# AILab-CVC/SEED-X

Measured on AMD Instinct MI355X. Metric: end-to-end generations/sec (img-in -> txt + 1024px-img-out), higher is better.
Workload: dtype fp16

## Files before the change

### include/seedx_hip.h

```cpp
#ifndef SEEDX_HIP_H
#define SEEDX_HIP_H
#include <stdint.h>
#ifdef __cplusplus
extern "C" {
#endif

#define SX_OK 0
#define SX_ERR_INVALID 1
#define SX_ERR_HIP 2

#define SX_F16 0
#define SX_BF16 1
#define SX_F32 2
#define SX_BF16X3 3
#define SX_F16X2 4
#define SX_FP8_E4M3 5
#define SX_FP4_E2M1 6
#define SX_TILED16 0x100

#define SX_ACT_NONE 0
#define SX_ACT_GELU 1
#define SX_ACT_SILU 2

#define SX_A_LINEAR 0
// ... 8 lines not shown
  void* C;
  const float* bias;
  const float* bias2d;
  const float* residual;
  int32_t M, N, K;
  int32_t ldc, ldr;
  int32_t n_valid;
  int32_t res_mod;
  int32_t bias2d_rows;
  int32_t dtype;
  int32_t out_dtype;
  int32_t act;
  int32_t glu;
  int32_t a_mode;
  int32_t B, Hin, Win, Cin, Hout, Wout;
  int32_t stride;
  int32_t upsample;
  int32_t ld_bias2d;
  int32_t pad_mode;
  int32_t a_planes;
} sx_gemm_args;
int sx_gemm(const sx_gemm_args* args, void* stream);
int sx_gemm_gn(const sx_gemm_args* args, double* stats, int groups, int rows_per_sample, int* fused_host, void* stream);
typedef struct sx_gemm_ln_args {
  void* x16_out;
  double* row_stats_out;
  const double* row_stats_in;
  const float* colsum;
  int32_t ld_x16;
  int32_t dim;
  float eps;
  int32_t reserved;
} sx_gemm_ln_args;
int sx_gemm_ln(const sx_gemm_args* args, const sx_gemm_ln_args* ln, void* stream);
int sx_gemm_force_tile(int cfg);
int sx_gemm_debug_stamps(void* buf);
int sx_gemm_pick_tile(int M, int N, int K, int glu, int conv);

typedef struct sx_gemv_args {
  const void* x;
  const void* W;
  void* y;
  const float* residual;
  int32_t M, N, K;
  int32_t dtype, out_dtype, act, glu;
  int32_t w_layout;
// ... 346 lines not shown
```

### seed-x_amd/_lib.py

```python
import ctypes as C
import os

_HERE = os.path.dirname(os.path.abspath(__file__))
LIB_PATH = os.path.join(_HERE, "lib", "libseedx_hip.so")

SX_F16, SX_BF16, SX_F32 = 0, 1, 2
SX_BF16X3 = 3
SX_F16X2 = 4
SX_FP8_E4M3 = 5
SX_FP4_E2M1 = 6
SX_TILED16 = 0x100
SX_ACT_NONE, SX_ACT_GELU, SX_ACT_SILU = 0, 1, 2
SX_A_LINEAR, SX_A_CONV3X3 = 0, 1

c_i32, c_i64, c_f32, c_vp = C.c_int32, C.c_int64, C.c_float, C.c_void_p


class GemmArgs(C.Structure):
    _fields_ = [("A", c_vp), ("W", c_vp), ("C", c_vp), ("bias", c_vp), ("bias2d", c_vp), ("residual", c_vp),
                ("M", c_i32), ("N", c_i32), ("K", c_i32), ("ldc", c_i32), ("ldr", c_i32), ("n_valid", c_i32),
                ("res_mod", c_i32), ("bias2d_rows", c_i32), ("dtype", c_i32), ("out_dtype", c_i32),
                ("act", c_i32), ("glu", c_i32), ("a_mode", c_i32),
                ("B", c_i32), ("Hin", c_i32), ("Win", c_i32), ("Cin", c_i32), ("Hout", c_i32), ("Wout", c_i32),
                ("stride", c_i32), ("upsample", c_i32), ("ld_bias2d", c_i32), ("pad_mode", c_i32), ("a_planes", c_i32)]
# ... 92 lines not shown
    _fields_ = [("Q", c_vp), ("K", c_vp), ("V", c_vp), ("O", c_vp),
                ("B", c_i32), ("H", c_i32), ("Sq", c_i32), ("Skv", c_i32), ("D", c_i32), ("reserved", c_i32),
                ("q_batch_stride", c_i64), ("q_row_stride", c_i64), ("q_head_stride", c_i64),
                ("k_batch_stride", c_i64), ("k_row_stride", c_i64), ("k_head_stride", c_i64),
                ("v_batch_stride", c_i64), ("v_row_stride", c_i64), ("v_head_stride", c_i64),
                ("o_batch_stride", c_i64), ("o_row_stride", c_i64),
                ("scale", c_f32), ("causal", c_i32), ("dtype", c_i32)]


class AttnSmallArgs(C.Structure):
    _fields_ = [("Q", c_vp), ("K", c_vp), ("V", c_vp), ("O", c_vp),
                ("B", c_i32), ("H", c_i32), ("Sq", c_i32), ("Skv", c_i32), ("D", c_i32),
                ("q_batch_stride", c_i64), ("q_row_stride", c_i64), ("q_head_stride", c_i64),
                ("k_batch_stride", c_i64), ("k_row_stride", c_i64), ("k_head_stride", c_i64),
                ("v_batch_stride", c_i64), ("v_row_stride", c_i64), ("v_head_stride", c_i64),
                ("o_batch_stride", c_i64), ("o_row_stride", c_i64),
                ("scale", c_f32), ("dtype", c_i32)]


SIGNATURES = {
    "sx_version": [],
    "sx_gemm": [C.POINTER(GemmArgs), c_vp],
    "sx_gemm_gn": [C.POINTER(GemmArgs), c_vp, c_i32, c_i32, C.POINTER(c_i32), c_vp],
    "sx_gemm_ln": [C.POINTER(GemmArgs), C.POINTER(GemmLnArgs), c_vp],
    "sx_gemm_force_tile": [c_i32],
    "sx_gemm_debug_stamps": [c_vp],
    "sx_gemm_pick_tile": [c_i32, c_i32, c_i32, c_i32, c_i32],
    "sx_gemv": [C.POINTER(GemvArgs), c_vp],
    "sx_gemv_ssq_parts": [c_i32, c_i32, c_i32],
    "sx_gemv_plan": [C.POINTER(GemvArgs), C.POINTER(c_i32)],
    "sx_gemv_force_valu": [c_i32],
    "sx_layernorm": [c_vp, c_i32, c_vp, c_i32, c_vp, c_vp, c_i32, c_i32, c_f32, c_i32, c_vp],
    "sx_softmax_rows": [c_vp, c_i64, c_vp, c_i64, c_i32, c_i32, c_f32, c_i32, c_vp],
    "sx_groupnorm": [c_vp, c_vp, c_vp, c_i32, c_vp, c_vp, c_vp, c_i32, c_i32, c_i32, c_i32, c_f32, c_i32, c_vp],
    "sx_groupnorm2": [c_vp, c_vp, c_i32, c_vp, c_vp, c_i32, c_vp, c_vp, c_vp, c_i32, c_i32, c_i32, c_i32, c_f32, c_i32, c_vp],
    "sx_groupnorm_sp": [c_vp, c_vp, c_i32, c_vp, c_vp, c_i32, c_vp, c_vp, c_vp, c_i32, c_i32, c_i32, c_i32, c_i32, c_f32, c_i32,
                        c_i32, c_vp],
    "sx_attention": [C.POINTER(AttnArgs), c_vp],
    "sx_norm_tune": [c_i32, c_i32],
    "sx_gemv_tune": [c_i32, c_i32],
    "sx_comm_alloc": [C.POINTER(c_vp), C.c_uint64],
    "sx_comm_free": [c_vp],
    "sx_ipc_export": [c_vp, C.c_char_p],
    "sx_ipc_open": [C.c_char_p, C.POINTER(c_vp)],
    "sx_ipc_close": [c_vp],
    "sx_allreduce_oneshot": [C.POINTER(OneshotArgs), c_vp],
# ... 94 lines not shown
```

### seed-x_amd/csrc/gemm.hip

```cpp
#include "gemm_common.h"

namespace sxk_gemm {

template <typename TT, int BM, int BN, int WM, int WN, int NSTAGE, int AMODE>
__global__ __launch_bounds__(WM * WN * 64) void gemm_kernel(const GemmP p) {
#if defined(__HIP_DEVICE_COMPILE__)
  typedef typename TT::vec8 vec8;
  constexpr int NW = WM * WN;
  static_assert(NW == 4 || NW == 8, "4 or 8 waves per block");
  constexpr int TM = BM / WM, TN = BN / WN;
  constexpr int FM = TM / 16, FN = TN / 16;
  constexpr bool kGlu = (FN % 2 == 0);
  constexpr int BNP = (BN + 8 * NW - 1) / (8 * NW) * (8 * NW);
  constexpr int A_PER_WAVE = BM / (8 * NW);
  constexpr int B_PER_WAVE = BNP / (8 * NW);
  constexpr int LOADS = A_PER_WAVE + B_PER_WAVE;
  constexpr int A_BYTES = BM * 128, B_BYTES = BNP * 128, STAGE = A_BYTES + B_BYTES;
  static_assert(LOADS * (NSTAGE - 1) <= 63, "vmcnt range");
  extern __shared__ __attribute__((aligned(16))) unsigned char smem[];

  const int tid = threadIdx.x, lane = tid & 63;
  const int wave = __builtin_amdgcn_readfirstlane(tid >> 6);
  const int wm = wave / WN, wn = wave % WN;
  unsigned long long t_start = 0, t_first = 0, t_main = 0;
// ... 377 lines not shown
  GemmP p;
  memset(&p, 0, sizeof(p));
  p.A = a->A; p.W = a->W; p.C = a->C; p.bias = a->bias; p.bias2d = a->bias2d; p.residual = a->residual;
  SX_CHECK(a->a_planes >= 0 && a->a_planes <= 2, "sx_gemm: a_planes=%d", a->a_planes);
  const int planes = a->a_planes == 2 ? 2 : 1;
  SX_CHECK(planes == 1 || (a->a_mode == SX_A_LINEAR && !ln), "sx_gemm: a_planes = 2 is for plain linear GEMMs");
  const int Kk = a->K * planes;
  p.M = a->M; p.N = a->N; p.K = Kk; p.Kw = a->K; p.ldc = a->ldc; p.ldr = a->ldr; p.res_mod = a->res_mod;
  p.n_valid = a->n_valid > 0 ? a->n_valid : n_out;
  p.bias2d_rows = a->bias2d_rows; p.out_dtype = a->out_dtype; p.act = a->act; p.glu = a->glu;
  p.ldb2 = a->ld_bias2d > 0 ? a->ld_bias2d : a->N;
  p.pad = 1;
  uint64_t a_bytes;
  const bool phases = a->a_mode == SX_A_CONV3X3 && a->upsample == 2;
  if (a->a_mode == SX_A_CONV3X3) {
    SX_CHECK(a->upsample >= 0 && a->upsample <= 2, "sx_gemm conv: upsample=%d", a->upsample);
    SX_CHECK(a->Cin % 64 == 0 && a->K == (phases ? 4 : 9) * a->Cin, "sx_gemm conv: Cin=%d K=%d", a->Cin, a->K);
    SX_CHECK(a->stride == 1 || a->stride == 2, "sx_gemm conv: stride");
    if (phases) {
      SX_CHECK(a->stride == 1 && a->pad_mode == 0, "sx_gemm conv: upsample = 2 is stride 1, pad 1");
      SX_CHECK((int64_t)a->B * a->Hin * a->Win % 256 == 0,
               "sx_gemm conv: upsample = 2 needs B*Hin*Win %% 256 == 0 (B=%d Hin=%d Win=%d): a 256-row tile must not straddle a phase",
               a->B, a->Hin, a->Win);
      SX_CHECK(!a->residual && !gn_stats, "sx_gemm conv: upsample = 2 takes no residual and no GroupNorm statistics");
    }
    SX_CHECK(a->M == a->B * a->Hout * a->Wout, "sx_gemm conv: M != B*Hout*Wout");
    const int hv = a->upsample ? 2 * a->Hin : a->Hin, wv = a->upsample ? 2 * a->Win : a->Win;
    SX_CHECK(a->pad_mode == 0 || a->pad_mode == 1, "sx_gemm conv: pad_mode");
    const int padsum = a->pad_mode ? 1 : 2;
    SX_CHECK(a->Hout == (hv + padsum - 3) / a->stride + 1 && a->Wout == (wv + padsum - 3) / a->stride + 1,
             "sx_gemm conv: output geometry mismatch");
    p.pad = a->pad_mode ? 0 : 1;
    p.Hin = a->Hin; p.Win = a->Win; p.Cin = a->Cin; p.Hout = a->Hout; p.Wout = a->Wout;
    p.stride = a->stride; p.upsample = a->upsample;
    a_bytes = (uint64_t)a->B * a->Hin * a->Win * a->Cin * 2;
  } else {
    SX_CHECK(a->a_mode == SX_A_LINEAR, "sx_gemm: bad a_mode");
    a_bytes = (uint64_t)a->M * Kk * 2;
  }
  const uint64_t w_bytes = (uint64_t)a->N * a->K * 2 * (phases ? 4 : 1);
  SX_CHECK(a_bytes < 0x7fffffffull && w_bytes < 0x7fffffffull, "sx_gemm: operand exceeds 2 GiB descriptor range");
  p.a_bytes = (unsigned)a_bytes;
  p.w_bytes = (unsigned)w_bytes;
  hipStream_t st = (hipStream_t)stream;
  p.res_init = (p.residual && p.act == SX_ACT_NONE && !p.glu) ? 1 : 0;
  if (ln) {
    SX_CHECK(a->a_mode == SX_A_LINEAR && !gn_stats, "sx_gemm_ln: linear GEMMs only");
// ... 6 lines not shown
    } else {
      SX_CHECK(ln->colsum && ln->dim == a->K && ln->eps > 0.f, "sx_gemm_ln consumer: colsum / dim (= K) / eps");
      SX_CHECK(a->out_dtype == a->dtype && !a->residual && !a->bias2d, "sx_gemm_ln consumer: 16-bit output, no residual / bias2d");
      p.ln_in = ln->row_stats_in; p.ln_cs = ln->colsum; p.ln_eps = ln->eps; p.ln_inv_dim = 1.0f / (float)ln->dim;
    }
  }
  unsigned allow = 0x7f;
  if (ln || phases) allow = 0;
  allow |= pp_supported(p, a->dtype, 256, a->a_mode) ? 0x80u : 0u;
  allow |= pp_supported(p, a->dtype, 320, a->a_mode) ? 0x100u : 0u;
  SX_CHECK(!(g_force_tile == 7 || g_force_tile == 8) || ((allow >> g_force_tile) & 1u),
           "sx_gemm: forced ping-pong tile has no kernel for this epilogue");
  if (ln) {
    const int plain = pick_tile(a->M, a->N, Kk, a->glu != 0, false, g_force_tile, 0x1ff);
    SX_CHECK((plain == 7 || plain == 8) && ((allow >> plain) & 1u),
             "sx_gemm_ln: M=%d N=%d K=%d does not run on a ping-pong tile with this epilogue (tile %d): keep sx_layernorm for it", a->M,
             a->N, a->K, plain);
    allow = 1u << plain;
  }
  SX_CHECK(!phases || allow, "sx_gemm conv: upsample = 2 has no ping-pong kernel for this epilogue");
  const int force = (phases && g_force_tile != 7 && g_force_tile != 8) ? -1 : g_force_tile;
  const int cfg = pick_tile(a->M, a->N, Kk, a->glu != 0, a->a_mode == SX_A_CONV3X3, force, allow);
  if (cfg == 7 || cfg == 8) {
    if (gn_stats && a->out_dtype == SX_F32 && !a->glu && a->act == SX_ACT_NONE && p.n_valid == a->N && a->N % gn_groups == 0 &&
        (a->N / gn_groups) % 2 == 0 && gn_rows % 256 == 0 && a->M % gn_rows == 0) {
      p.gn_stats = gn_stats; p.gn_groups = gn_groups; p.gn_cpg = a->N / gn_groups; p.gn_rows = gn_rows;
      *gn_fused = 1;
    }
    return launch_pp(p, a->dtype, cfg == 7 ? 256 : 320, a->a_mode, st);
  }
#define SX_GEMM_DISPATCH(TT)                                                  \
  switch (cfg) {                                                              \
    case 0: return launch_cfg<TT, 128, 128, 2, 2, 2>(p, a->a_mode, st);       \
    case 1: return launch_cfg<TT, 128, 80, 4, 1, 3>(p, a->a_mode, st);        \
    case 2: return launch_cfg<TT, 64, 128, 2, 2, 3>(p, a->a_mode, st);        \
    case 3: return launch_cfg<TT, 64, 64, 2, 2, 3>(p, a->a_mode, st);         \
    case 4: return launch_cfg<TT, 256, 256, 2, 4, 2>(p, a->a_mode, st);       \
    case 5: return launch_cfg<TT, 256, 320, 2, 4, 2>(p, a->a_mode, st);       \
    default: return launch_cfg<TT, 256, 160, 4, 2, 2>(p, a->a_mode, st);      \
  }
  if (a->dtype == SX_BF16) { SX_GEMM_DISPATCH(BF16) } else { SX_GEMM_DISPATCH(F16) }
#undef SX_GEMM_DISPATCH
}
```

### seed-x_amd/csrc/gemm_pp.hip

```cpp
#include "gemm_common.h"
#include <type_traits>

namespace sxk_gemm {

#define SX_A_CONV3X3_UP 2
#define SX_A_CONV3X3_PH 3

#define PP_SYNC()                            \
  do {                                       \
    __builtin_amdgcn_sched_barrier(0);       \
    __builtin_amdgcn_s_barrier();            \
    __builtin_amdgcn_sched_barrier(0);       \
  } while (0)

template <typename TT, int BN, int AMODE, bool OUT32, int ACT, bool GLU, int LN = 0>
__global__ __launch_bounds__(512) void gemm_pp_kernel(const GemmP p) {
#if defined(__HIP_DEVICE_COMPILE__)
  typedef typename TT::vec8 vec8;
  static_assert(LN != 2 || (OUT32 && !GLU && ACT == SX_ACT_NONE), "the LayerNorm producer is the plain fp32-output epilogue");
  constexpr int BM = 256, TN = BN / 4, FN = TN / 16, FM = 8, FH = 4;
  constexpr int NB = BN / 64;
  constexpr int C1 = NB - 3, C2 = 3;
  constexpr int WAITN = 4 + NB;
  constexpr int A_BYTES = BM * 128, STAGE = A_BYTES + BN * 128;
// ... 442 lines not shown
      x += __builtin_bit_cast(float, __builtin_amdgcn_update_dpp(0, __builtin_bit_cast(int, x), 0x140, 0xF, 0xF, true));
      return x;
    };
#pragma unroll
    for (int i = 0; i < FN; ++i) {
      gsl[i] = row16_sum(gsl[i]);
      gql[i] = row16_sum(gql[i]);
      gsh[i] = row16_sum(gsh[i]);
      gqh[i] = row16_sum(gqh[i]);
    }
    float* gslot = (float*)smem;
    const int gbase = n0 / p.gn_cpg;
    const int nlast = (n0 + BN < p.N ? n0 + BN : p.N) - 1;
    const int ngr = nlast / p.gn_cpg - gbase + 1;
    __syncthreads();
    if ((lane & 15) == 0) {
#pragma unroll
      for (int i = 0; i < FN; ++i) {
        const int cp = (wc * TN + i * 16 + lq) >> 1;
        *(f32x4_t*)(gslot + ((size_t)g * (BN / 2) + cp) * 2) = (f32x4_t){gsl[i], gql[i], gsh[i], gqh[i]};
      }
    }
    __syncthreads();
    const int smp = m0 / p.gn_rows;
    for (int t = tid; t < 2 * ngr; t += 512) {
      const int G = gbase + (t >> 1), which = t & 1;
      int c_lo = G * p.gn_cpg - n0, c_hi = (G + 1) * p.gn_cpg - n0;
      c_lo = c_lo < 0 ? 0 : c_lo;
      const int c_end = (p.N - n0 < BN ? p.N - n0 : BN);
      c_hi = c_hi > c_end ? c_end : c_hi;
      float acc = 0.f;
      for (int cp = c_lo >> 1; cp < (c_hi >> 1); ++cp) acc += gslot[(size_t)cp * 2 + which];
      for (int cp = c_lo >> 1; cp < (c_hi >> 1); ++cp) acc += gslot[((size_t)(BN / 2) + cp) * 2 + which];
      atomicAdd(&p.gn_stats[((size_t)smp * p.gn_groups + G) * 2 + which], (double)acc);
    }
  }
  if (p.dbg) {
    asm volatile("s_waitcnt vmcnt(0)" ::: "memory");
    const unsigned long long t_end = __builtin_amdgcn_s_memtime();
    if (tid == 0) {
      unsigned long long* d = p.dbg + (size_t)blockIdx.x * 4;
      d[0] = t_start; d[1] = t_first; d[2] = t_main; d[3] = t_end;
    }
  }
#endif
}

// ... 128 lines not shown
```

### seed-x_amd/ops.py

```python
import contextlib
import ctypes as C
import gc
import math

import os

import torch

from . import _lib
from ._lib import (SX_A_CONV3X3, SX_A_LINEAR, SX_ACT_GELU, SX_ACT_NONE, SX_ACT_SILU, SX_BF16, SX_F16, SX_F32,
                   AttnArgs, AttnSmallArgs, GemmArgs, GemvArgs, check)

_DT = {torch.float16: SX_F16, torch.bfloat16: SX_BF16, torch.float32: SX_F32}
_TD = {v: k for k, v in _DT.items()}
ACT = {None: SX_ACT_NONE, "none": SX_ACT_NONE, "gelu": SX_ACT_GELU, "silu": SX_ACT_SILU}


def dt_code(dtype):
    return _DT[dtype]


def _stream():
    return C.c_void_p(torch.cuda.current_stream().cuda_stream)

# ... 7 lines not shown


@contextlib.contextmanager
def graph_capture(g):
    gc.collect()
    was = gc.isenabled()
    gc.disable()
    try:
        with torch.cuda.graph(g):
            yield
    finally:
        if was:
            gc.enable()


def _f32c(t):
    if t is None:
        return None
    assert t.dtype == torch.float32 and t.is_contiguous(), "expected contiguous fp32 tensor"
    return t


class GnStats:
    __slots__ = ("buf", "groups", "rows", "ready")

    def __init__(self, buf, groups, rows):
        self.buf, self.groups, self.rows, self.ready = buf, int(groups), int(rows), False

    @staticmethod
    def arena(n, B, groups, device):
        return torch.zeros((n, B, groups, 2), dtype=torch.float64, device=device)


class LnRows:
    __slots__ = ("x16", "stats")

    def __init__(self, M, C, dtype, device, stats=None):
        self.x16 = torch.empty((M, C), dtype=dtype, device=device)
        self.stats = stats if stats is not None else torch.zeros((M, 2), dtype=torch.float64, device=device)
        assert self.stats.shape == (M, 2) and self.stats.dtype == torch.float64 and self.stats.is_contiguous()


def gemm_tile(M, N, K, glu=False, conv=False):
    return int(_lib.load().sx_gemm_pick_tile(int(M), int(N), int(K), 1 if glu else 0, 1 if conv else 0))


def ln_fold_ok(M, C, consumers, producers):
    return all(gemm_tile(M, n, C, glu) >= 7 for n, glu in consumers) and all(gemm_tile(M, C, k) >= 7 for k in producers)


def fold_layernorm(w, bias, gamma, beta):
    wf = (w.float() * gamma.float()[None, :]).to(w.dtype).contiguous()
    cs = wf.float().sum(dim=1).contiguous()
    b = w.float() @ beta.float()
    if bias is not None:
        b = b + bias.float()
    return wf, cs, b.contiguous()


GN_FUSE = os.environ.get("SX_GN_FUSE", "1") != "0"


def _launch_gemm(lib, args, gn, what):
    if gn is None or not GN_FUSE:
        check(lib.sx_gemm(C.byref(args), _stream()), what)
        return
    assert gn.buf.dtype == torch.float64 and gn.buf.is_contiguous() and args.M % gn.rows == 0 \
        and gn.buf.numel() == (args.M // gn.rows) * gn.groups * 2, "GnStats does not describe this output"
    fused = C.c_int32(0)
    check(lib.sx_gemm_gn(C.byref(args), gn.buf.data_ptr(), gn.groups, gn.rows, C.byref(fused), _stream()), what)
    gn.ready = bool(fused.value)


def gemm(a, w, bias=None, bias2d=None, bias2d_rows=0, residual=None, res_mod=0, act=None, glu=False,
         out_dtype=None, out=None, n_valid=0, ld_bias2d=0, gn=None, ln_emit=None, ln_apply=None, a_planes=1):
    lib = _lib.load()
    assert a.dim() == 2 and w.dim() == 2 and a.is_contiguous() and w.is_contiguous()
    assert a.dtype == w.dtype and a.dtype in (torch.float16, torch.bfloat16)
    M, K = a.shape
    N = w.shape[0]
    assert a_planes in (1, 2) and K % a_planes == 0
    K //= a_planes
    assert w.shape[1] == K, f"K mismatch {a.shape} vs {w.shape} (a_planes {a_planes})"
# ... 54 lines not shown
            for ky in kys:
                for kx in kxs:
                    wp[2 * a + c, :, u, v] += w9[:, ky, kx]
    if not rounded:
        assert planes == 1
        return wp.view(4, Cout, 4 * C)
    if planes == 1:
        return wp.to(dtype or w.dtype).view(4, Cout, 4 * C).contiguous()
    s32 = wp.float()
    hi = s32.to(torch.bfloat16)
    lo = (s32 - hi.float()).to(torch.bfloat16)
    return torch.cat([hi, lo, hi], dim=4).view(4, Cout, 12 * C).contiguous()


def upsample_phases_ok(B, H, W):
    return (B * H * W) % 256 == 0


def conv3x3(x, w, bias=None, bias2d=None, residual=None, stride=1, upsample=False, out_dtype=None, act=None,
            n_valid=0, pad_mode=0, gn=None, w_phases=None, out=None):
    lib = _lib.load()
    assert x.dim() == 4 and x.is_contiguous()
    B, H, W, Cin = x.shape
    phases = (w_phases is not None and upsample and stride == 1 and pad_mode == 0 and residual is None and gn is None
              and act is None and upsample_phases_ok(B, H, W))
    if phases:
        assert w_phases.dim() == 3 and w_phases.shape[0] == 4 and w_phases.shape[2] == 4 * Cin and w_phases.dtype == x.dtype
        w = w_phases
        Cout, K = w.shape[1], 4 * Cin
    else:
        assert w is not None, "conv3x3: this call needs the 36-tap weight (the phase gate does not hold)"
        Cout, K = w.shape
        assert K == 9 * Cin
    assert w.is_contiguous()
    hv, wv = (2 * H, 2 * W) if upsample else (H, W)
    padsum = 1 if pad_mode else 2
    Hout, Wout = (hv + padsum - 3) // stride + 1, (wv + padsum - 3) // stride + 1
    M = B * Hout * Wout
    out_dtype = out_dtype or x.dtype
    n_store = n_valid if n_valid else Cout
    if out is None:
        out = torch.empty((M, n_store), dtype=out_dtype, device=x.device)
    assert out.shape == (M, n_store) and out.dtype == out_dtype and out.is_contiguous()
    args = GemmArgs()
    args.A, args.W, args.C = x.data_ptr(), w.data_ptr(), out.data_ptr()
    args.bias = _f32c(bias).data_ptr() if bias is not None else None
    args.n_valid = n_valid
# ... 252 lines not shown
    return gemm(x, w, **kw)


def layernorm(x, gamma, beta, eps, out_dtype, rms=False, tiled=False):
    lib = _lib.load()
    assert x.is_contiguous()
    cols = x.shape[-1]
    rows = x.numel() // cols
    if tiled:
        yt = Tiled16(rows, cols, out_dtype, x.device)
        y, code = yt.t, _DT[out_dtype] | _lib.SX_TILED16
    else:
        y, code = torch.empty(x.shape, dtype=out_dtype, device=x.device), _DT[out_dtype]
    check(lib.sx_layernorm(_p(x), _DT[x.dtype], _p(y), code, _p(_f32c(gamma)), _p(_f32c(beta)), rows, cols,
                           float(eps), 1 if rms else 0, _stream()), "sx_layernorm")
    return yt if tiled else y


def rmsnorm(x, gamma, eps, out_dtype, tiled=False):
    return layernorm(x, gamma, None, eps, out_dtype, rms=True, tiled=tiled)


def groupnorm(x, gamma, beta, groups, eps, silu, out_dtype, want_raw=False, x2=None, comm=None, hw_total=None, planes=False,
              stats=None):
    lib = _lib.load()
    assert x.dtype == torch.float32 and x.is_contiguous() and x.dim() == 3
    B, HW, C1 = x.shape
    Cc = C1
    if x2 is not None:
        assert x2.dtype == torch.float32 and x2.is_contiguous() and x2.shape[:2] == (B, HW)
        Cc = C1 + x2.shape[2]
    if planes == 2:
        out_dtype, code, cols = torch.float16, _lib.SX_F16X2, 2 * Cc
    elif planes:
        out_dtype, code, cols = torch.bfloat16, _lib.SX_BF16X3, 3 * Cc
    else:
        code, cols = _DT[out_dtype], Cc
    y = torch.empty((B, HW, cols), dtype=out_dtype, device=x.device)
    raw = torch.empty((B, HW, cols), dtype=out_dtype, device=x.device) if want_raw else None
    if stats is not None and stats.ready and x2 is None and (comm is None or comm.world == 1):
        assert stats.groups == groups and stats.rows == HW and stats.buf.numel() == B * groups * 2
        check(lib.sx_groupnorm_sp(_p(x), None, C1, _p(y), _p(raw), code, _p(_f32c(gamma)), _p(_f32c(beta)), _p(stats.buf), B, HW, HW,
                                  Cc, groups, float(eps), 1 if silu else 0, 2, _stream()), "sx_groupnorm_sp(apply, fused statistics)")
        return (y, raw) if want_raw else y
    stats = torch.empty((B, groups, 2), dtype=torch.float64, device=x.device)
    if comm is None or comm.world == 1:
        check(lib.sx_groupnorm2(_p(x), _p(x2), C1, _p(y), _p(raw), code, _p(_f32c(gamma)), _p(_f32c(beta)), _p(stats),
                                B, HW, Cc, groups, float(eps), 1 if silu else 0, _stream()), "sx_groupnorm")
    else:
        args = (_p(x), _p(x2), C1, _p(y), _p(raw), code, _p(_f32c(gamma)), _p(_f32c(beta)), _p(stats), B, HW,
                int(hw_total), Cc, groups, float(eps), 1 if silu else 0)
        check(lib.sx_groupnorm_sp(*args, 1, _stream()), "sx_groupnorm_sp(stats)")
        comm.all_reduce(stats)
        check(lib.sx_groupnorm_sp(*args, 2, _stream()), "sx_groupnorm_sp(apply)")
    return (y, raw) if want_raw else y


def softmax_rows(x, scale, out_dtype):
    lib = _lib.load()
    assert x.dtype == torch.float32 and x.dim() == 2 and x.stride(1) == 1
    R, Cc = x.shape
    y = torch.empty((R, Cc), dtype=out_dtype, device=x.device)
    check(lib.sx_softmax_rows(_p(x), x.stride(0), _p(y), y.stride(0), R, Cc, float(scale), _DT[out_dtype], _stream()),
          "sx_softmax_rows")
    return y


def _bshd_strides(t):
    assert t.dim() == 4 and t.stride(3) == 1, "expected a [B, S, H, D] view with unit stride on D"
    return t.stride(0), t.stride(1), t.stride(2)


def attention(q, k, v, scale, causal=False, out=None):
    lib = _lib.load()
    B, Sq, H, D = q.shape
    Skv = k.shape[1]
    assert k.shape == (B, Skv, H, D) and v.shape == (B, Skv, H, D) and q.dtype == k.dtype == v.dtype
    if out is None:
# ... 733 lines not shown
```

### seed-x_amd/unet.py

```python
import math
import os
import types

import torch

from . import ops
from .llama import glu_pack_rows

LN_FOLD = os.environ.get("SX_LN_FOLD", "1") != "0"

SDXL_BASE_CONFIG = dict(in_channels=4, out_channels=4, block_out_channels=(320, 640, 1280), layers_per_block=2,
                        down_attn=(False, True, True), up_attn=(True, True, False), transformer_layers=(1, 2, 10),
                        heads=(5, 10, 20), cross_attention_dim=2048, addition_time_embed_dim=256, pooled_dim=1280,
                        norm_groups=32, sample_size=128)


class UNetOutput:
    def __init__(self, sample):
        self.sample = sample


class UNet2DConditionModel:
    def __init__(self, comm=None, **cfg):
        from .parallel import Comm
# ... 186 lines not shown
                n = f"up_blocks.{i}.upsamplers.0.conv"
                blk["up"] = (conv16(n + ".weight"), f32(n + ".bias"))
                w = sd[n + ".weight"].detach().to(dev)
                blk["up_ph"] = ops.pack_upsample_phases(w.permute(0, 2, 3, 1).reshape(w.shape[0], -1), dtype=dt)
            P["up"].append(blk)
        P["norm_out"] = (f32("conv_norm_out.weight"), f32("conv_norm_out.bias"))
        wo = conv16("conv_out.weight")
        wop = torch.zeros(16, wo.shape[1], dtype=dt, device=dev)
        wop[:wo.shape[0]] = wo
        bo = torch.zeros(16, dtype=torch.float32, device=dev)
        bo[:wo.shape[0]] = f32("conv_out.bias")
        P["conv_out_w"], P["conv_out_b"] = wop, bo
        ws = [sd[n + ".time_emb_proj.weight"].detach().to(dev, dt) for n in self._temb_names]
        bs = [sd[n + ".time_emb_proj.bias"].detach().to(dev, torch.float32) for n in self._temb_names]
        P["temb_w"], P["temb_b"] = torch.cat(ws, 0).contiguous(), torch.cat(bs, 0).contiguous()
        off, P["temb_off"] = 0, {}
        for n, w_ in zip(self._temb_names, ws):
            P["temb_off"][n] = (off, w_.shape[0])
            off += w_.shape[0]
        self._P = P
        self._sd = None
        return P

    def _gn(self, x, gb, eps, silu, Hc, Wc, want_raw=False, x2=None, stats=None):
        G, dt = self.cfg["norm_groups"], self.dtype
        return ops.groupnorm(x, gb[0], gb[1], G, eps, silu, dt, want_raw=want_raw, x2=x2, comm=self.comm, hw_total=Hc * Wc,
                             stats=stats)

    def _gn_slot(self, B, HW):
        if self._gn_arena is None:
            return None
        i = self._gn_next
        self._gn_next += 1
        if i >= self._gn_arena.shape[0]:
            return None
        return ops.GnStats(self._gn_arena[i], self.cfg["norm_groups"], HW)

    def _conv(self, h16, B, Hc, Wc, w, bias=None, bias2d=None, residual=None, stride=1, upsample=False, n_valid=0, gn=None,
              w_phases=None):
        tp = self.comm.world
        Cin = h16.shape[-1]
        if tp == 1:
            return ops.conv3x3(h16.view(B, Hc, Wc, Cin), w, bias=bias, bias2d=bias2d, residual=residual, stride=stride,
                               upsample=upsample, out_dtype=torch.float32, n_valid=n_valid, gn=gn, w_phases=w_phases)
        from . import seqpar
        Hl = Hc // tp
        Co = n_valid or w.shape[0]
        if stride == 2:
            xin = seqpar.with_halo(h16, self.comm, Hl, Wc, left_col=True, bottom=False)
            out = ops.conv3x3(xin, w, bias=bias, bias2d=bias2d, stride=2, pad_mode=1, out_dtype=torch.float32)
            assert residual is None
            return out.view(B, (Hl // 2) * (Wc // 2), Co)
        xin = seqpar.with_halo(h16, self.comm, Hl, Wc)
        out = ops.conv3x3(xin, w, bias=bias, bias2d=bias2d, upsample=upsample, out_dtype=torch.float32, n_valid=n_valid)
        f = 2 if upsample else 1
        out = out.view(B, f * (Hl + 2), f * Wc, Co)[:, f:f * (Hl + 1)].reshape(B, f * Hl * f * Wc, Co).contiguous()
        if residual is not None:
            out = ops.add(out, residual.reshape(out.shape).contiguous())
        return out

    def _resnet(self, r, x, B, Hc, Wc, temb_all, skip=None, st_in=None):
        Ci = x.shape[-1] + (skip.shape[-1] if skip is not None else 0)
        if "ws" in r:
            h, raw = self._gn(x, r["n1"], 1e-5, True, Hc, Wc, want_raw=True, x2=skip)
        else:
            assert skip is None
            h = self._gn(x, r["n1"], 1e-5, True, Hc, Wc, stats=st_in)
        off, Co = self._P["temb_off"][r["name"]]
        HW = x.shape[1]
        st2 = self._gn_slot(B, HW)
        h = self._conv(h, B, Hc, Wc, r["w1"], bias=r["b1"], bias2d=temb_all[:, off:off + Co], gn=st2)
        h = self._gn(h, r["n2"], 1e-5, True, Hc, Wc, stats=st2)
        if "ws" in r:
            sc = ops.gemm(raw.view(-1, Ci), r["ws"], bias=r["bs"], out_dtype=torch.float32)
        else:
            sc = x.view(-1, Ci)
        st_out = self._gn_slot(B, HW)
        out = self._conv(h, B, Hc, Wc, r["w2"], bias=r["b2"], residual=sc, gn=st_out).view(B, -1, Co)
        self._mark(out)
        return out, st_out

    def _transformer(self, t, x, B, ctx_kv, Hc, Wc, st_in=None):
        dt, heads = self.dtype, t["heads"]
        _, HW, C = x.shape
        hd = C // heads
        scale = hd ** -0.5
        sp = self.comm.world > 1
        h = self._gn(x, t["norm"], 1e-6, False, Hc, Wc, stats=st_in)
        nb = len(t["blocks"])
        M = B * HW
        if LN_FOLD and not sp and "f1" in t["blocks"][0] and self._ln_fold_ok(M, C):
            arena = torch.zeros((3 * nb, M, 2), dtype=torch.float64, device=x.device)

            def rows(i):
                return ops.LnRows(M, C, dt, x.device, stats=arena[i])
            ln = rows(0)
            hs = ops.gemm(h.view(-1, C), t["pin_w"], bias=t["pin_b"], out_dtype=torch.float32, ln_emit=ln)
            for k, b in enumerate(t["blocks"]):
                w, cs, bb = b["f1"]
                qkv = ops.gemm(ln.x16, w, bias=bb, ln_apply=(ln, cs, 1e-5)).view(B, HW, 3, heads, hd)
                att = ops.attention(qkv[:, :, 0], qkv[:, :, 1], qkv[:, :, 2], scale)
                ln = rows(3 * k + 1)
                hs = ops.gemm(att.view(-1, C), b["wo1"], bias=b["bo1"], residual=hs, out_dtype=torch.float32, ln_emit=ln)
                self._mark(hs)
                w, cs, bb = b["f2"]
                q = ops.gemm(ln.x16, w, bias=bb, ln_apply=(ln, cs, 1e-5)).view(B, HW, heads, hd)
                kv = ctx_kv[k]
                att = ops.attention(q, kv[:, :, 0], kv[:, :, 1], scale)
                ln = rows(3 * k + 2)
                hs = ops.gemm(att.view(-1, C), b["wo2"], bias=b["bo2"], residual=hs, out_dtype=torch.float32, ln_emit=ln)
                w, cs, bb = b["f3"]
                g = ops.gemm(ln.x16, w, bias=bb, act="gelu", glu=True, ln_apply=(ln, cs, 1e-5))
                if k == nb - 1:
                    hs = ops.gemm(g, b["wff2"], bias=b["bff2"], residual=hs, out_dtype=dt)
                else:
                    ln = rows(3 * k + 3)
                    hs = ops.gemm(g, b["wff2"], bias=b["bff2"], residual=hs, out_dtype=torch.float32, ln_emit=ln)
                self._mark(hs)
            st_out = self._gn_slot(B, HW)
            out = ops.gemm(hs, t["pout_w"], bias=t["pout_b"], residual=x.view(-1, C), out_dtype=torch.float32, gn=st_out)
            return out.view(B, HW, C), st_out
        hs = ops.gemm(h.view(-1, C), t["pin_w"], bias=t["pin_b"], out_dtype=torch.float32)
        for k, b in enumerate(t["blocks"]):
            n = ops.layernorm(hs, b["n1"][0], b["n1"][1], 1e-5, dt)
            if not sp:
                qkv = ops.gemm(n, b["wqkv"]).view(B, HW, 3, heads, hd)
                att = ops.attention(qkv[:, :, 0], qkv[:, :, 1], qkv[:, :, 2], scale)
            else:
                from . import seqpar
                kv_l = ops.gemm(n, b["wqkv"][C:]).view(B, HW, 2, heads, hd)
                pending = self.comm.all_gather_async(kv_l)
                q = ops.gemm(n, b["wqkv"][:C]).view(B, HW, heads, hd)
                g = pending.wait()
                kv = g.permute(1, 0, 2, 3, 4, 5).reshape(B, g.shape[0] * HW, 2, heads, hd).contiguous()
                att = ops.attention(q, kv[:, :, 0], kv[:, :, 1], scale)
            hs = ops.gemm(att.view(-1, C), b["wo1"], bias=b["bo1"], residual=hs, out_dtype=torch.float32)
            self._mark(hs)
            n = ops.layernorm(hs, b["n2"][0], b["n2"][1], 1e-5, dt)
            q = ops.gemm(n, b["wq2"]).view(B, HW, heads, hd)
            kv = ctx_kv[k]
            att = ops.attention(q, kv[:, :, 0], kv[:, :, 1], scale)
            hs = ops.gemm(att.view(-1, C), b["wo2"], bias=b["bo2"], residual=hs, out_dtype=torch.float32)
            n = ops.layernorm(hs, b["n3"][0], b["n3"][1], 1e-5, dt)
            g = ops.gemm(n, b["wff1"], bias=b["bff1"], act="gelu", glu=True)
            last = k == nb - 1
            hs = ops.gemm(g, b["wff2"], bias=b["bff2"], residual=hs, out_dtype=dt if last else torch.float32)
            self._mark(hs)
        st_out = self._gn_slot(B, HW)
        out = ops.gemm(hs, t["pout_w"], bias=t["pout_b"], residual=x.view(-1, C), out_dtype=torch.float32, gn=st_out)
        return out.view(B, HW, C), st_out

    def _ln_fold_ok(self, M, C):
        key = (M, C)
        if key not in self._ln_ok:
            self._ln_ok[key] = ops.ln_fold_ok(M, C, consumers=[(3 * C, False), (C, False), (8 * C, True)], producers=[C, 4 * C])
        return self._ln_ok[key]

    def prepare_context(self, encoder_hidden_states):
        P = self._pack()
        ehs = encoder_hidden_states
        key = (ehs.data_ptr(), ehs._version, tuple(ehs.shape))
        if self._ctx_key == key:
            return self._ctx
        B, L, ca = ehs.shape
        e16 = ops.cast(ehs.to(self.device).float().contiguous(), self.dtype).view(B * L, ca)
        ctx = []
        for t in self._xattn:
            heads = t["heads"]
            per = []
            for b in t["blocks"]:
                C = b["wq2"].shape[0]
# ... 12 lines not shown
        tid = ops.timestep_embedding(time_ids.reshape(-1).float().contiguous(), c["addition_time_embed_dim"], torch.float32)
        add = torch.empty((B, self.add_embedding.linear_1.in_features), dtype=torch.float32, device=self.device)
        ops.copy2d(text_embeds.float().contiguous(), add, 0)
        ops.copy2d(tid.view(B, -1), add, text_embeds.shape[1])
        a = ops.gemm(ops.cast(add, dt), P["ae1"][0], bias=P["ae1"][1], act="silu")
        emb = ops.gemm(a, P["ae2"][0], bias=P["ae2"][1], residual=e, out_dtype=torch.float32)
        return ops.gemm(ops.silu_cast(emb, dt), P["temb_w"], bias=P["temb_b"], out_dtype=torch.float32)

    def _mark(self, t=None):
        if self._trace is not None and t is not None:
            self._trace.append(t.detach().float().clone())
        if self._on_mark is not None:
            self._mark_i += 1
            self._on_mark(self._mark_i)

    def forward_nhwc(self, x_in, temb_all, ctx, B, H, W, on_mark=None):
        P, dt, c = self._P, self.dtype, self.cfg
        self._on_mark, self._mark_i = on_mark, 0
        cin = c["in_channels"]
        tp, rank = self.comm.world, self.comm.rank
        if tp > 1:
            from . import seqpar
            assert H % (tp * 4) == 0, f"latent rows {H} must divide by 4 x the sharding degree {tp} (two 2x down-samplings)"
        col = ops.im2col3x3_small(x_in.view(B, H, W, cin), self.cin_kpad, dt)
        x = ops.gemm(col, P["conv_in_w"], bias=P["conv_in_b"], out_dtype=torch.float32).view(B, H * W, -1)
        if tp > 1:
            x = seqpar.local_rows(x, rank, tp, H, W)
        skips = [(x, H, W)]
        ti = 0
        Hc, Wc = H, W
        self._gn_arena = ops.GnStats.arena(self._n_gn_slots, B, c["norm_groups"], x.device) if tp == 1 else None
        self._gn_next = 0
        st = None
        for blk in P["down"]:
            for j, r in enumerate(blk["res"]):
                x, st = self._resnet(r, x, B, Hc, Wc, temb_all, st_in=st)
                if blk["attn"]:
                    x, st = self._transformer(blk["attn"][j], x, B, ctx[ti], Hc, Wc, st_in=st)
                    ti += 1
                skips.append((x, Hc, Wc))
            if blk["down"] is not None:
                st = self._gn_slot(B, (Hc // 2) * (Wc // 2))
                x = self._conv(ops.cast(x, dt), B, Hc, Wc, blk["down"][0], bias=blk["down"][1], stride=2, gn=st)
                Hc, Wc = Hc // 2, Wc // 2
                skips.append((x, Hc, Wc))
        x, st = self._resnet(P["mid"]["res"][0], x, B, Hc, Wc, temb_all, st_in=st)
        x, st = self._transformer(P["mid"]["attn"][0], x, B, ctx[ti], Hc, Wc, st_in=st)
        ti += 1
        x, st = self._resnet(P["mid"]["res"][1], x, B, Hc, Wc, temb_all, st_in=st)
        for blk in P["up"]:
            for j, r in enumerate(blk["res"]):
                s, _, _ = skips.pop()
                x, st = self._resnet(r, x.contiguous(), B, Hc, Wc, temb_all, skip=s)
                if blk["attn"]:
                    x, st = self._transformer(blk["attn"][j], x, B, ctx[ti], Hc, Wc, st_in=st)
                    ti += 1
            if blk["up"] is not None:
                x = self._conv(ops.cast(x, dt), B, Hc, Wc, blk["up"][0], bias=blk["up"][1], upsample=True, w_phases=blk["up_ph"])
                Hc, Wc = Hc * 2, Wc * 2
                st = None
        h = self._gn(x, P["norm_out"], 1e-5, True, Hc, Wc, stats=st)
        self._gn_arena = None
        self._on_mark = None
        nv = 4 if c["out_channels"] == 4 else 0
        out = self._conv(h, B, Hc, Wc, P["conv_out_w"], bias=P["conv_out_b"], n_valid=nv)
        out = out.view(B, -1, out.shape[-1])
        if tp > 1:
            out = seqpar.gather_rows(out, self.comm)
            if not torch.cuda.is_current_stream_capturing():
                self.comm.check()
        return out

    def forward(self, sample, timestep, encoder_hidden_states, added_cond_kwargs=None, cross_attention_kwargs=None,
                return_dict=True, **_):
        self._pack()
        assert added_cond_kwargs is not None and "text_embeds" in added_cond_kwargs and "time_ids" in added_cond_kwargs
        B, Cin, H, W = sample.shape
        assert Cin == self.cfg["in_channels"]
        dev = self.device
        t = torch.as_tensor(timestep, dtype=torch.float32, device=dev).reshape(-1)
        t = t.expand(B).contiguous() if t.numel() == 1 else t
        temb = self.time_embeddings(t, None, added_cond_kwargs["text_embeds"].to(dev), added_cond_kwargs["time_ids"].to(dev), B)
        ctx = self.prepare_context(encoder_hidden_states.to(dev))
# ... 9 lines not shown
```

Measured before the change: 1.361.

## Emit per-cell GroupNorm statistics from GEMM epilogues and regroup them for skip concatenation

GroupNorm statistics are now accumulated in finer channel cells (C/64 or C/32 wide) inside GEMM and conv epilogues. A small regroup kernel merges these cells into the real group statistics, which also works when a skip tensor is concatenated, so the up-block ResNets no longer need a separate statistics pass. The fused statistics path is also enabled for the phase-decomposed upsample convolution and for conv_in. The goal is to drop the standalone GroupNorm reduction passes over large activations. In exchange it adds an extra tiny kernel per norm, makes slot and arena bookkeeping more complex, and risks wrong sample indexing in the phase-conv path.

```diff
diff --git a/include/seedx_hip.h b/include/seedx_hip.h
--- a/include/seedx_hip.h
+++ b/include/seedx_hip.h
@@ -54,6 +54,9 @@
 } sx_gemm_args;
 int sx_gemm(const sx_gemm_args* args, void* stream);
 int sx_gemm_gn(const sx_gemm_args* args, double* stats, int groups, int rows_per_sample, int* fused_host, void* stream);
+int sx_gn_cell_width(int C);
+int sx_gn_regroup(const double* cells1, int C1, int cell1, const double* cells2, int C2, int cell2, double* stats, int B, int groups,
+                  void* stream);
 typedef struct sx_gemm_ln_args {
   void* x16_out;
   double* row_stats_out;
diff --git a/seed-x_amd/_lib.py b/seed-x_amd/_lib.py
--- a/seed-x_amd/_lib.py
+++ b/seed-x_amd/_lib.py
@@ -138,6 +138,8 @@
     "sx_version": [],
     "sx_gemm": [C.POINTER(GemmArgs), c_vp],
     "sx_gemm_gn": [C.POINTER(GemmArgs), c_vp, c_i32, c_i32, C.POINTER(c_i32), c_vp],
+    "sx_gn_cell_width": [c_i32],
+    "sx_gn_regroup": [c_vp, c_i32, c_i32, c_vp, c_i32, c_i32, c_vp, c_i32, c_i32, c_vp],
     "sx_gemm_ln": [C.POINTER(GemmArgs), C.POINTER(GemmLnArgs), c_vp],
     "sx_gemm_force_tile": [c_i32],
     "sx_gemm_debug_stamps": [c_vp],
diff --git a/seed-x_amd/csrc/gemm.hip b/seed-x_amd/csrc/gemm.hip
--- a/seed-x_amd/csrc/gemm.hip
+++ b/seed-x_amd/csrc/gemm.hip
@@ -423,7 +423,7 @@
       SX_CHECK((int64_t)a->B * a->Hin * a->Win % 256 == 0,
                "sx_gemm conv: upsample = 2 needs B*Hin*Win %% 256 == 0 (B=%d Hin=%d Win=%d): a 256-row tile must not straddle a phase",
                a->B, a->Hin, a->Win);
-      SX_CHECK(!a->residual && !gn_stats, "sx_gemm conv: upsample = 2 takes no residual and no GroupNorm statistics");
+      SX_CHECK(!a->residual, "sx_gemm conv: upsample = 2 takes no residual");
     }
     SX_CHECK(a->M == a->B * a->Hout * a->Wout, "sx_gemm conv: M != B*Hout*Wout");
     const int hv = a->upsample ? 2 * a->Hin : a->Hin, wv = a->upsample ? 2 * a->Win : a->Win;
@@ -476,8 +476,10 @@
   const int force = (phases && g_force_tile != 7 && g_force_tile != 8) ? -1 : g_force_tile;
   const int cfg = pick_tile(a->M, a->N, Kk, a->glu != 0, a->a_mode == SX_A_CONV3X3, force, allow);
   if (cfg == 7 || cfg == 8) {
+    const bool gn_geom = gn_stats && (phases ? (gn_rows == a->Hout * a->Wout && (a->Hin * a->Win) % 256 == 0)
+                                             : (gn_rows % 256 == 0 && a->M % gn_rows == 0));
     if (gn_stats && a->out_dtype == SX_F32 && !a->glu && a->act == SX_ACT_NONE && p.n_valid == a->N && a->N % gn_groups == 0 &&
-        (a->N / gn_groups) % 2 == 0 && gn_rows % 256 == 0 && a->M % gn_rows == 0) {
+        (a->N / gn_groups) % 2 == 0 && gn_geom) {
       p.gn_stats = gn_stats; p.gn_groups = gn_groups; p.gn_cpg = a->N / gn_groups; p.gn_rows = gn_rows;
       *gn_fused = 1;
     }
diff --git a/seed-x_amd/csrc/gemm_pp.hip b/seed-x_amd/csrc/gemm_pp.hip
--- a/seed-x_amd/csrc/gemm_pp.hip
+++ b/seed-x_amd/csrc/gemm_pp.hip
@@ -488,7 +488,7 @@
       }
     }
     __syncthreads();
-    const int smp = m0 / p.gn_rows;
+    const int smp = (AMODE == SX_A_CONV3X3_PH) ? (m0 - ph * (p.M >> 2)) / (p.gn_rows >> 2) : m0 / p.gn_rows;
     for (int t = tid; t < 2 * ngr; t += 512) {
       const int G = gbase + (t >> 1), which = t & 1;
       int c_lo = G * p.gn_cpg - n0, c_hi = (G + 1) * p.gn_cpg - n0;
diff --git a/seed-x_amd/csrc/gn_cells.hip b/seed-x_amd/csrc/gn_cells.hip
--- /dev/null
+++ b/seed-x_amd/csrc/gn_cells.hip
@@ -0,0 +1,52 @@
+#include "sx_common.h"
+
+namespace sxk_cells {
+
+__global__ __launch_bounds__(256) void cells_regroup_kernel(const double* c1, int C1, int w1, const double* c2, int C2, int w2,
+                                                            double* out, int B, int groups) {
+  const int t = blockIdx.x * 256 + threadIdx.x;
+  if (t >= B * groups * 2) return;
+  const int which = t & 1, g = (t >> 1) % groups, b = (t >> 1) / groups;
+  const int gw = (C1 + C2) / groups;
+  const int lo = g * gw, hi = lo + gw;
+  double acc = 0.0;
+  const int n1 = C1 / w1;
+  const int a_hi = hi < C1 ? hi : C1;
+  for (int c = lo / w1; c * w1 < a_hi; ++c) acc += c1[((size_t)b * n1 + c) * 2 + which];
+  if (c2 && hi > C1) {
+    const int n2 = C2 / w2;
+    const int b_lo = (lo > C1 ? lo : C1) - C1, b_hi = hi - C1;
+    for (int c = b_lo / w2; c * w2 < b_hi; ++c) acc += c2[((size_t)b * n2 + c) * 2 + which];
+  }
+  out[t] = acc;
+}
+
+}
+
+extern "C" int sx_gn_cell_width(int C) {
+  if (C <= 0) return 0;
+  if (C % 64 == 0 && (C / 64) % 2 == 0) return C / 64;
+  if (C % 32 == 0 && (C / 32) % 2 == 0) return C / 32;
+  return 0;
+}
+
+extern "C" int sx_gn_regroup(const double* cells1, int C1, int cell1, const double* cells2, int C2, int cell2, double* stats, int B,
+                             int groups, void* stream) {
+  SX_CHECK(cells1 && stats && B > 0 && groups > 0, "sx_gn_regroup: null pointer / empty problem");
+  SX_CHECK(C1 > 0 && cell1 > 0 && cell1 % 2 == 0 && C1 % cell1 == 0, "sx_gn_regroup: C1=%d cell1=%d (cells are even and divide C1)", C1,
+           cell1);
+  if (!cells2) C2 = 0;
+  SX_CHECK(!cells2 || (C2 > 0 && cell2 > 0 && cell2 % 2 == 0 && C2 % cell2 == 0),
+           "sx_gn_regroup: C2=%d cell2=%d (cells are even and divide C2)", C2, cell2);
+  const int C = C1 + C2;
+  SX_CHECK(C % groups == 0, "sx_gn_regroup: C=%d groups=%d", C, groups);
+  const int gw = C / groups;
+  SX_CHECK(gw % cell1 == 0, "sx_gn_regroup: groups of %d channels do not end on the first source's %d-channel cells", gw, cell1);
+  SX_CHECK(!cells2 || (gw % cell2 == 0 && C1 % cell2 == 0),
+           "sx_gn_regroup: groups of %d channels behind %d do not end on the second source's %d-channel cells", gw, C1, cell2);
+  const int n = B * groups * 2;
+  hipLaunchKernelGGL(sxk_cells::cells_regroup_kernel, dim3((n + 255) / 256), dim3(256), 0, (hipStream_t)stream, cells1, C1, cell1,
+                     cells2, C2, cell2 > 0 ? cell2 : 2, stats, B, groups);
+  SX_HIP_LAUNCH_CHECK();
+  return SX_OK;
+}
diff --git a/seed-x_amd/ops.py b/seed-x_amd/ops.py
--- a/seed-x_amd/ops.py
+++ b/seed-x_amd/ops.py
@@ -53,14 +53,40 @@
 
 
 class GnStats:
-    __slots__ = ("buf", "groups", "rows", "ready")
-
-    def __init__(self, buf, groups, rows):
-        self.buf, self.groups, self.rows, self.ready = buf, int(groups), int(rows), False
+    __slots__ = ("buf", "groups", "rows", "ready", "cell")
+
+    def __init__(self, buf, groups, rows, cell=0):
+        self.buf, self.groups, self.rows, self.ready, self.cell = buf, int(groups), int(rows), False, int(cell)
 
     @staticmethod
     def arena(n, B, groups, device):
         return torch.zeros((n, B, groups, 2), dtype=torch.float64, device=device)
+
+    @staticmethod
+    def cells(slot, B, C, rows):
+        w = gn_cell_width(C)
+        if not w or slot.numel() < B * (C // w) * 2:
+            return None
+        return GnStats(slot.view(-1)[:B * (C // w) * 2].view(B, C // w, 2), C // w, rows, cell=w)
+
+
+def gn_cell_width(C):
+    for n in (64, 32):
+        if C > 0 and C % n == 0 and (C // n) % 2 == 0:
+            return C // n
+    return 0
+
+
+def gn_cells_ok(groups, C1, cell1, C2=0, cell2=0):
+    C = C1 + C2
+    if groups <= 0 or C % groups or cell1 <= 0 or cell1 % 2 or C1 % cell1:
+        return False
+    gw = C // groups
+    if gw % cell1:
+        return False
+    if C2:
+        return cell2 > 0 and cell2 % 2 == 0 and C2 % cell2 == 0 and gw % cell2 == 0 and C1 % cell2 == 0
+    return True
 
 
 class LnRows:
@@ -90,6 +116,7 @@
 
 
 GN_FUSE = os.environ.get("SX_GN_FUSE", "1") != "0"
+GN_CELLS = os.environ.get("SX_GN_CELLS", "1") != "0"
 
 
 def _launch_gemm(lib, args, gn, what):
@@ -190,7 +217,8 @@
     lib = _lib.load()
     assert x.dim() == 4 and x.is_contiguous()
     B, H, W, Cin = x.shape
-    phases = (w_phases is not None and upsample and stride == 1 and pad_mode == 0 and residual is None and gn is None
+    phases = (w_phases is not None and upsample and stride == 1 and pad_mode == 0 and residual is None
+              and (gn is None or (GN_CELLS and (H * W) % 256 == 0))
               and act is None and upsample_phases_ok(B, H, W))
     if phases:
         assert w_phases.dim() == 3 and w_phases.shape[0] == 4 and w_phases.shape[2] == 4 * Cin and w_phases.dtype == x.dtype
@@ -489,7 +517,7 @@
 
 
 def groupnorm(x, gamma, beta, groups, eps, silu, out_dtype, want_raw=False, x2=None, comm=None, hw_total=None, planes=False,
-              stats=None):
+              stats=None, stats2=None):
     lib = _lib.load()
     assert x.dtype == torch.float32 and x.is_contiguous() and x.dim() == 3
     B, HW, C1 = x.shape
@@ -505,11 +533,24 @@
         code, cols = _DT[out_dtype], Cc
     y = torch.empty((B, HW, cols), dtype=out_dtype, device=x.device)
     raw = torch.empty((B, HW, cols), dtype=out_dtype, device=x.device) if want_raw else None
-    if stats is not None and stats.ready and x2 is None and (comm is None or comm.world == 1):
+    single = comm is None or comm.world == 1
+    if stats is not None and stats.ready and not stats.cell and x2 is None and single:
         assert stats.groups == groups and stats.rows == HW and stats.buf.numel() == B * groups * 2
         check(lib.sx_groupnorm_sp(_p(x), None, C1, _p(y), _p(raw), code, _p(_f32c(gamma)), _p(_f32c(beta)), _p(stats.buf), B, HW, HW,
                                   Cc, groups, float(eps), 1 if silu else 0, 2, _stream()), "sx_groupnorm_sp(apply, fused statistics)")
         return (y, raw) if want_raw else y
+    srcs = [stats] if x2 is None else [stats, stats2]
+    if GN_CELLS and single and all(s is not None and s.ready and s.cell for s in srcs):
+        s2 = srcs[1] if x2 is not None else None
+        if gn_cells_ok(groups, C1, stats.cell, Cc - C1, s2.cell if s2 else 0):
+            for s, c in zip(srcs, (C1, Cc - C1)):
+                assert s.rows == HW and s.groups * s.cell == c and s.buf.numel() == B * s.groups * 2 and s.buf.is_contiguous()
+            st = torch.empty((B, groups, 2), dtype=torch.float64, device=x.device)
+            check(lib.sx_gn_regroup(_p(stats.buf), C1, stats.cell, _p(s2.buf) if s2 else None, Cc - C1, s2.cell if s2 else 0, _p(st),
+                                    B, groups, _stream()), "sx_gn_regroup")
+            check(lib.sx_groupnorm_sp(_p(x), _p(x2), C1, _p(y), _p(raw), code, _p(_f32c(gamma)), _p(_f32c(beta)), _p(st), B, HW, HW,
+                                      Cc, groups, float(eps), 1 if silu else 0, 2, _stream()), "sx_groupnorm_sp(apply, cell statistics)")
+            return (y, raw) if want_raw else y
     stats = torch.empty((B, groups, 2), dtype=torch.float64, device=x.device)
     if comm is None or comm.world == 1:
         check(lib.sx_groupnorm2(_p(x), _p(x2), C1, _p(y), _p(raw), code, _p(_f32c(gamma)), _p(_f32c(beta)), _p(stats),
@@ -521,6 +562,16 @@
         comm.all_reduce(stats)
         check(lib.sx_groupnorm_sp(*args, 2, _stream()), "sx_groupnorm_sp(apply)")
     return (y, raw) if want_raw else y
+
+
+def gn_cells_pass(x, st):
+    lib = _lib.load()
+    assert x.dtype == torch.float32 and x.is_contiguous() and x.dim() == 3 and st.cell and not st.ready
+    B, HW, C_ = x.shape
+    assert st.rows == HW and st.groups * st.cell == C_ and st.buf.numel() == B * st.groups * 2 and st.buf.is_contiguous()
+    check(lib.sx_groupnorm_sp(_p(x), None, C_, None, None, _lib.SX_F32, None, None, _p(st.buf), B, HW, HW, C_, st.groups, 1e-5, 0, 1,
+                              _stream()), "sx_groupnorm_sp(statistics of cells)")
+    st.ready = True
 
 
 def softmax_rows(x, scale, out_dtype):
diff --git a/seed-x_amd/unet.py b/seed-x_amd/unet.py
--- a/seed-x_amd/unet.py
+++ b/seed-x_amd/unet.py
@@ -232,19 +232,24 @@
         self._sd = None
         return P
 
-    def _gn(self, x, gb, eps, silu, Hc, Wc, want_raw=False, x2=None, stats=None):
+    def _gn(self, x, gb, eps, silu, Hc, Wc, want_raw=False, x2=None, stats=None, stats2=None):
         G, dt = self.cfg["norm_groups"], self.dtype
         return ops.groupnorm(x, gb[0], gb[1], G, eps, silu, dt, want_raw=want_raw, x2=x2, comm=self.comm, hw_total=Hc * Wc,
-                             stats=stats)
-
-    def _gn_slot(self, B, HW):
+                             stats=stats, stats2=stats2)
+
+    def _gn_slot(self, B, HW, C=None):
         if self._gn_arena is None:
             return None
         i = self._gn_next
         self._gn_next += 1
         if i >= self._gn_arena.shape[0]:
             return None
-        return ops.GnStats(self._gn_arena[i], self.cfg["norm_groups"], HW)
+        G = self.cfg["norm_groups"]
+        if C is not None and ops.GN_CELLS:
+            st = ops.GnStats.cells(self._gn_arena[i], B, C, HW)
+            if st is not None:
+                return st
+        return ops.GnStats(self._gn_arena[i].view(-1)[:B * G * 2].view(B, G, 2), G, HW)
 
     def _conv(self, h16, B, Hc, Wc, w, bias=None, bias2d=None, residual=None, stride=1, upsample=False, n_valid=0, gn=None,
               w_phases=None):
@@ -269,10 +274,10 @@
             out = ops.add(out, residual.reshape(out.shape).contiguous())
         return out
 
-    def _resnet(self, r, x, B, Hc, Wc, temb_all, skip=None, st_in=None):
+    def _resnet(self, r, x, B, Hc, Wc, temb_all, skip=None, st_in=None, st_skip=None):
         Ci = x.shape[-1] + (skip.shape[-1] if skip is not None else 0)
         if "ws" in r:
-            h, raw = self._gn(x, r["n1"], 1e-5, True, Hc, Wc, want_raw=True, x2=skip)
+            h, raw = self._gn(x, r["n1"], 1e-5, True, Hc, Wc, want_raw=True, x2=skip, stats=st_in, stats2=st_skip)
         else:
             assert skip is None
             h = self._gn(x, r["n1"], 1e-5, True, Hc, Wc, stats=st_in)
@@ -285,7 +290,7 @@
             sc = ops.gemm(raw.view(-1, Ci), r["ws"], bias=r["bs"], out_dtype=torch.float32)
         else:
             sc = x.view(-1, Ci)
-        st_out = self._gn_slot(B, HW)
+        st_out = self._gn_slot(B, HW, Co)
         out = self._conv(h, B, Hc, Wc, r["w2"], bias=r["b2"], residual=sc, gn=st_out).view(B, -1, Co)
         self._mark(out)
         return out, st_out
@@ -327,7 +332,7 @@
                     ln = rows(3 * k + 3)
                     hs = ops.gemm(g, b["wff2"], bias=b["bff2"], residual=hs, out_dtype=torch.float32, ln_emit=ln)
                 self._mark(hs)
-            st_out = self._gn_slot(B, HW)
+            st_out = self._gn_slot(B, HW, C)
             out = ops.gemm(hs, t["pout_w"], bias=t["pout_b"], residual=x.view(-1, C), out_dtype=torch.float32, gn=st_out)
             return out.view(B, HW, C), st_out
         hs = ops.gemm(h.view(-1, C), t["pin_w"], bias=t["pin_b"], out_dtype=torch.float32)
@@ -356,7 +361,7 @@
             last = k == nb - 1
             hs = ops.gemm(g, b["wff2"], bias=b["bff2"], residual=hs, out_dtype=dt if last else torch.float32)
             self._mark(hs)
-        st_out = self._gn_slot(B, HW)
+        st_out = self._gn_slot(B, HW, C)
         out = ops.gemm(hs, t["pout_w"], bias=t["pout_b"], residual=x.view(-1, C), out_dtype=torch.float32, gn=st_out)
         return out.view(B, HW, C), st_out
 
@@ -415,43 +420,46 @@
         if tp > 1:
             from . import seqpar
             assert H % (tp * 4) == 0, f"latent rows {H} must divide by 4 x the sharding degree {tp} (two 2x down-samplings)"
+        slot_w = max(c["norm_groups"], 64) if ops.GN_CELLS else c["norm_groups"]
+        self._gn_arena = ops.GnStats.arena(self._n_gn_slots, B, slot_w, x_in.device) if tp == 1 else None
+        self._gn_next = 0
         col = ops.im2col3x3_small(x_in.view(B, H, W, cin), self.cin_kpad, dt)
-        x = ops.gemm(col, P["conv_in_w"], bias=P["conv_in_b"], out_dtype=torch.float32).view(B, H * W, -1)
+        st = self._gn_slot(B, H * W, P["conv_in_w"].shape[0]) if ops.GN_CELLS else None
+        x = ops.gemm(col, P["conv_in_w"], bias=P["conv_in_b"], out_dtype=torch.float32, gn=st).view(B, H * W, -1)
+        if st is not None and st.cell and not st.ready and ops.GN_FUSE:
+            ops.gn_cells_pass(x, st)
         if tp > 1:
             x = seqpar.local_rows(x, rank, tp, H, W)
-        skips = [(x, H, W)]
+        skips = [(x, st)]
         ti = 0
         Hc, Wc = H, W
-        self._gn_arena = ops.GnStats.arena(self._n_gn_slots, B, c["norm_groups"], x.device) if tp == 1 else None
-        self._gn_next = 0
-        st = None
         for blk in P["down"]:
             for j, r in enumerate(blk["res"]):
                 x, st = self._resnet(r, x, B, Hc, Wc, temb_all, st_in=st)
                 if blk["attn"]:
                     x, st = self._transformer(blk["attn"][j], x, B, ctx[ti], Hc, Wc, st_in=st)
                     ti += 1
-                skips.append((x, Hc, Wc))
+                skips.append((x, st))
             if blk["down"] is not None:
-                st = self._gn_slot(B, (Hc // 2) * (Wc // 2))
+                st = self._gn_slot(B, (Hc // 2) * (Wc // 2), blk["down"][0].shape[0])
                 x = self._conv(ops.cast(x, dt), B, Hc, Wc, blk["down"][0], bias=blk["down"][1], stride=2, gn=st)
                 Hc, Wc = Hc // 2, Wc // 2
-                skips.append((x, Hc, Wc))
+                skips.append((x, st))
         x, st = self._resnet(P["mid"]["res"][0], x, B, Hc, Wc, temb_all, st_in=st)
         x, st = self._transformer(P["mid"]["attn"][0], x, B, ctx[ti], Hc, Wc, st_in=st)
         ti += 1
         x, st = self._resnet(P["mid"]["res"][1], x, B, Hc, Wc, temb_all, st_in=st)
         for blk in P["up"]:
             for j, r in enumerate(blk["res"]):
-                s, _, _ = skips.pop()
-                x, st = self._resnet(r, x.contiguous(), B, Hc, Wc, temb_all, skip=s)
+                s, st_s = skips.pop()
+                x, st = self._resnet(r, x.contiguous(), B, Hc, Wc, temb_all, skip=s, st_in=st, st_skip=st_s)
                 if blk["attn"]:
                     x, st = self._transformer(blk["attn"][j], x, B, ctx[ti], Hc, Wc, st_in=st)
                     ti += 1
             if blk["up"] is not None:
-                x = self._conv(ops.cast(x, dt), B, Hc, Wc, blk["up"][0], bias=blk["up"][1], upsample=True, w_phases=blk["up_ph"])
+                st = self._gn_slot(B, 4 * Hc * Wc, blk["up"][0].shape[0]) if ops.GN_CELLS and (Hc * Wc) % 256 == 0 else None
+                x = self._conv(ops.cast(x, dt), B, Hc, Wc, blk["up"][0], bias=blk["up"][1], upsample=True, w_phases=blk["up_ph"], gn=st)
                 Hc, Wc = Hc * 2, Wc * 2
-                st = None
         h = self._gn(x, P["norm_out"], 1e-5, True, Hc, Wc, stats=st)
         self._gn_arena = None
         self._on_mark = None
```

Result: no change. 1.370, median of 6 (+0.6%).
